# shinshoji01/Style-Restricted_GAN

Hardware: AMD Instinct MI355X
Metric: images/sec G+D+E train step, CelebA 128x128 bs=32/GPU (higher is better)
Workload: dtype f32; 1 GPU; SRGAN-nopretrain (03-train) G+D+E train step, 128x128, bs=32/GPU, k=5, fp32, E trainable (BASELINE configs[1]); global_batch=32, unrolled_k=5, parallelism=dp1, graph_fallback=False, graph_segments=1, ranks_seen=1, execution=hipGraph replay of the captured step

## Files before the change

include/srgan_hip.h:

```cpp
#ifndef SRGAN_HIP_H
#define SRGAN_HIP_H

#include <stddef.h>
#include <stdint.h>

#ifdef __cplusplus
extern "C" {
#endif

#define SRGAN_ABI_VERSION 1

enum { SRGAN_ACT_NONE = 0, SRGAN_ACT_RELU = 1, SRGAN_ACT_LRELU = 2 };
enum { SRGAN_PAD_ZERO = 0, SRGAN_PAD_REFLECT = 1 };
enum { SRGAN_CRIT_MSE = 0, SRGAN_CRIT_BCE = 1 };

int srgan_abi_version(void);
const char* srgan_last_error(void);

typedef struct srgan_conv_desc {
  int N, Hi, Wi, I;
  int Ho, Wo, O;
  int kh, kw, stride, pad;
  int pad_mode;
  long long sO, sI, sH, sW;
// ... 152 lines not shown
                       void* dst, int dst_bf16, int act, float slope, void* ws, size_t ws_bytes, void* stream);
int srgan_igemm16_wgrad(const srgan_conv_desc* d, const void* x, const void* dy, float* dw, void* ws, size_t ws_bytes, void* stream);
int srgan_conv2d_io_applicable(const srgan_conv_desc* d, int act);
int srgan_conv2d_io_fwd(const srgan_conv_desc* d, const void* x, int x_bf16, const void* packed, const float* bias, void* y, int y_bf16,
                        int act, float slope, void* ws, size_t ws_bytes, void* stream);
int srgan_conv2d_io_dgrad(const srgan_conv_desc* d, const void* dy, int dy_bf16, const void* packed, void* dx, int dx_bf16, void* ws,
                          size_t ws_bytes, void* stream);
int srgan_act_bwd_io(const void* y, int y_bf16, const void* dy, int dy_bf16, void* dx, int dx_bf16, long long n, int act, float slope,
                     void* stream);
int srgan_instnorm_slab_applicable(int N, int HW, int C);
int srgan_instnorm_slab_fwd_io(const void* x, int x_bf16, const float* scale, const float* shift, const float* res, void* y,
                               int y_bf16, float* mean, float* rstd, int N, int HW, int C, float eps, int act, float slope,
                               void* stream);
int srgan_instnorm_slab_bwd_io(const void* x, int x_bf16, const void* dy, int dy_bf16, const float* scale, const float* shift,
                               const float* mean, const float* rstd, void* dx, int dx_bf16, float* dscale, float* dshift, int N,
                               int HW, int C, int act, float slope, void* stream);
int srgan_instnorm_io_applicable(int N, int HW, int C);
int srgan_instnorm_fwd_io(const void* x, int x_bf16, const float* scale, const float* shift, const float* res, void* y, int y_bf16,
                          float* mean, float* rstd, int N, int HW, int C, float eps, int act, float slope, void* ws, size_t ws_bytes,
                          void* stream);
int srgan_instnorm_bwd_io(const void* x, int x_bf16, const void* dy, int dy_bf16, const float* scale, const float* shift,
                          const float* mean, const float* rstd, void* dx, int dx_bf16, float* dscale, float* dshift, int N, int HW,
                          int C, int act, float slope, void* ws, size_t ws_bytes, void* stream);

int srgan_nchw_to_nhwc(const float* x, float* y, int N, int C, int H, int W, void* stream);
int srgan_nhwc_to_nchw(const float* x, float* y, int N, int C, int H, int W, void* stream);

int srgan_mse_const(const float* o, long long n, float target, float weight, float* loss, float* d_o, void* stream);
int srgan_crit_const(const float* o, long long n, float target, float weight, int kind, float* loss, float* d_o, void* stream);
int srgan_softmax_mse(const float* z, const long long* label, int B, int n_class, float weight,
                      float* q, float* loss, float* dz, void* stream);
int srgan_softmax_crit(const float* z, const long long* label, int B, int n_class, float weight, int kind,
                       float* q, float* loss, float* dz, void* stream);
int srgan_softmax_xent(const float* z, const long long* label, int B, int n_class, float weight, float* loss,
                       float* dz, void* stream);
size_t srgan_l1_workspace(long long n);
int srgan_l1_mean(const float* a, const float* b, long long n, float weight, float* loss,
                  float* da, float* db, void* ws, size_t ws_bytes, void* stream);
int srgan_latent_losses(const float* mu, int B, int d, float n_batch, const float* hist_target, int bins,
                        float range_max, float sigma, float w_bkl, float w_corr, float w_hist,
                        float* vals, float* dmu, float* corr_out , void* stream);
int srgan_d_losses(const float* const* o, const long long* per_row, const float* const* z, int n_scales, int rows,
                   int rows_first, int n_class, const long long* label, float t_first, float t_rest, float w_class,
                   float* vals, float* const* d_o, float* const* dz, void* stream);
int srgan_d_losses_crit(const float* const* o, const long long* per_row, const float* const* z, int n_scales, int rows,
                        int rows_first, int n_class, const long long* label, float t_first, float t_rest, float w_class,
// ... 87 lines not shown
```

style-restricted_gan_amd/csrc/norm.hip:

```cpp
#include <algorithm>
#include <cstdlib>
#include <cstring>
#include "common.h"

namespace srgan {

constexpr int NORM_CH = 32;
constexpr int NORM_ROWS = 8;

template <bool B16>
__device__ __forceinline__ f32x4 ld4(const void* base, size_t idx) {
  if constexpr (B16) return __builtin_convertvector(*reinterpret_cast<const bf16x4*>(static_cast<const __bf16*>(base) + idx), f32x4);
  else return *reinterpret_cast<const f32x4*>(static_cast<const float*>(base) + idx);
}
template <bool B16>
__device__ __forceinline__ void st4(void* base, size_t idx, f32x4 v) {
  if constexpr (B16) *reinterpret_cast<bf16x4*>(static_cast<__bf16*>(base) + idx) = __builtin_convertvector(v, bf16x4);
  else *reinterpret_cast<f32x4*>(static_cast<float*>(base) + idx) = v;
}


template <bool B16>
__device__ __forceinline__ void ld8(const void* base, size_t idx, f32x4& lo, f32x4& hi) {
  if constexpr (B16) {
// ... 277 lines not shown
  for (int s = 0; s < S; ++s) {
    const float2 p = part[((size_t)n * S + s) * C + c];
    a += p.x;
    b += p.y;
  }
  stats_finish(a, b, x[(size_t)n * HW * C + c], HW, eps, &mean[idx], &rstd[idx]);
}

__device__ __forceinline__ void sum_partials4(const float2* __restrict__ part, int n, int S, int C, int c, f32x4* a, f32x4* b) {
  f32x4 sa = {0.f, 0.f, 0.f, 0.f}, sb = {0.f, 0.f, 0.f, 0.f};
  for (int s = 0; s < S; ++s) {
    const f32x4* q = reinterpret_cast<const f32x4*>(part + ((size_t)n * S + s) * C + c);
    const f32x4 lo = q[0], hi = q[1];
    sa[0] += lo[0]; sb[0] += lo[1]; sa[1] += lo[2]; sb[1] += lo[3];
    sa[2] += hi[0]; sb[2] += hi[1]; sa[3] += hi[2]; sb[3] += hi[3];
  }
  *a = sa;
  *b = sb;
}

template <bool V4>
__global__ void in_apply(const float* __restrict__ x, const float* __restrict__ scale, const float* __restrict__ shift,
                         const float* __restrict__ res, const float* __restrict__ mean, const float* __restrict__ rstd,
                         float* __restrict__ y, long long total, int HWC, int C, int act, float slope) {
  constexpr int W = V4 ? 4 : 1;
  for (long long i = ((long long)blockIdx.x * blockDim.x + threadIdx.x) * W; i < total;
       i += (long long)gridDim.x * blockDim.x * W) {
    const int n = (int)(i / HWC);
    const int c = (int)(i % C);
    float xv[W], rv[W], o[W];
    if constexpr (V4) {
      *reinterpret_cast<f32x4*>(xv) = *reinterpret_cast<const f32x4*>(x + i);
      if (res) *reinterpret_cast<f32x4*>(rv) = *reinterpret_cast<const f32x4*>(res + i);
    } else {
      xv[0] = x[i];
      if (res) rv[0] = res[i];
    }
#pragma unroll
    for (int k = 0; k < W; ++k) {
      const int nc = n * C + c + k;
      float v = (xv[k] - mean[nc]) * rstd[nc];
      if (scale) v = v * scale[nc] + shift[nc];
      v = apply_act(v, act, slope);
      if (res) v += rv[k];
      o[k] = v;
    }
    if constexpr (V4) *reinterpret_cast<f32x4*>(y + i) = *reinterpret_cast<const f32x4*>(o);
    else y[i] = o[0];
  }
}

template <bool X16 = false, bool Y16 = false>
__global__ __launch_bounds__(256) void in_apply_pow2(const void* __restrict__ x, const float* __restrict__ scale,
                                                     const float* __restrict__ shift, const float* __restrict__ res,
                                                     float* __restrict__ mean, float* __restrict__ rstd,
                                                     void* __restrict__ y, int HWC4, int C, int act, float slope,
                                                     const float2* __restrict__ part, int S, int HW, float eps) {
  const int n = blockIdx.y;
  const int c = (threadIdx.x * 4) % C;
  const int nc = n * C + c;
  f32x4 mu, rs;
  if (part) {
    f32x4 a, b;
    sum_partials4(part, n, S, C, c, &a, &b);
    const f32x4 x0 = ld4<X16>(x, (size_t)n * HWC4 * 4 + c);
#pragma unroll
    for (int e = 0; e < 4; ++e) {
      float m1, r1;
      stats_finish(a[e], b[e], x0[e], HW, eps, &m1, &r1);
      mu[e] = m1;
      rs[e] = r1;
    }
    if (blockIdx.x == 0 && threadIdx.x * 4 < C) {
      *reinterpret_cast<f32x4*>(mean + nc) = mu;
      *reinterpret_cast<f32x4*>(rstd + nc) = rs;
    }
  } else {
    mu = *reinterpret_cast<const f32x4*>(mean + nc);
    rs = *reinterpret_cast<const f32x4*>(rstd + nc);
  }
  f32x4 sc = {1.f, 1.f, 1.f, 1.f}, sf = {0.f, 0.f, 0.f, 0.f};
  if (scale) {
    sc = *reinterpret_cast<const f32x4*>(scale + nc);
    sf = *reinterpret_cast<const f32x4*>(shift + nc);
  }
  const size_t base = (size_t)n * HWC4;
  const f32x4* rp = res ? reinterpret_cast<const f32x4*>(res) + base : nullptr;
  auto xat = [&](int j) __attribute__((always_inline)) { return ld4<X16>(x, (base + j) * 4); };
  auto yput = [&](int j, f32x4 v) __attribute__((always_inline)) { st4<Y16>(y, (base + j) * 4, v); };
  auto one = [&](f32x4 xv, f32x4 rv) __attribute__((always_inline)) {
    f32x4 v = ((xv - mu) * rs) * sc + sf;
#pragma unroll
    for (int k = 0; k < 4; ++k) v[k] = apply_act(v[k], act, slope);
    return rp ? v + rv : v;
  };
  const int step = gridDim.x * 256;
  int j = blockIdx.x * 256 + threadIdx.x;
  const f32x4 zero = {0.f, 0.f, 0.f, 0.f};
  for (; j + 3 * step < HWC4; j += 4 * step) {
    const f32x4 x0v = xat(j), x1v = xat(j + step), x2v = xat(j + 2 * step), x3v = xat(j + 3 * step);
    f32x4 r0 = zero, r1 = zero, r2 = zero, r3 = zero;
    if (rp) { r0 = rp[j]; r1 = rp[j + step]; r2 = rp[j + 2 * step]; r3 = rp[j + 3 * step]; }
    yput(j, one(x0v, r0));
    yput(j + step, one(x1v, r1));
    yput(j + 2 * step, one(x2v, r2));
    yput(j + 3 * step, one(x3v, r3));
  }
  for (; j < HWC4; j += step) yput(j, one(xat(j), rp ? rp[j] : zero));
}

template <bool X16 = false, bool G16 = false, bool D16 = false>
// ... 562 lines not shown
    else if (rows <= 2) SRGAN_FWD_SLAB(2);
    else if (rows <= 4) SRGAN_FWD_SLAB(4);
    else if (rows <= 8) SRGAN_FWD_SLAB(8);
    else SRGAN_FWD_SLAB(16);
#undef SRGAN_FWD_SLAB
    prof_end(tok, st);
    return check_launch("instnorm_fwd (slab)");
  }
  float2* part = reinterpret_cast<float2*>(ws);
  dim3 g((C + NORM_CH - 1) / NORM_CH, S, N);
  {
    ProfToken tok = prof_begin(30, tbytes, st);
    if ((C & 3) == 0) hipLaunchKernelGGL(in_stats_partial_v4<false>, g, dim3(256), 0, st, (const void*)x, part, HW, C, S, rps);
    else hipLaunchKernelGGL(in_stats_partial, g, dim3(256), 0, st, x, part, HW, C, S, rps);
    prof_end(tok, st);
  }
  const long long total = (long long)N * HW * C;
  const bool fuse_final = (const float*)y != x && (const float*)y != res;
  if (pow2_fast(C, HW) && fuse_final) {
    const int hwc4 = HW * C / 4;
    dim3 g2((unsigned)apply_grid(hwc4, N), (unsigned)N);
    ProfToken tok = prof_begin(31, (res ? 3.0 : 2.0) * tbytes, st);
    hipLaunchKernelGGL((in_apply_pow2<false, false>), g2, dim3(256), 0, st, (const void*)x, scale, shift, res, mean, rstd, (void*)y, hwc4, C, act, slope,
                       (const float2*)part, S, HW, eps);
    prof_end(tok, st);
    return check_launch("instnorm_fwd");
  }
  hipLaunchKernelGGL(in_stats_final, dim3((N * C + 255) / 256), dim3(256), 0, st, x, (const float2*)part, mean, rstd, N, HW, C, S, eps);
  if (pow2_fast(C, HW)) {
    const int hwc4 = HW * C / 4;
    dim3 g2((unsigned)apply_grid(hwc4, N), (unsigned)N);
    hipLaunchKernelGGL((in_apply_pow2<false, false>), g2, dim3(256), 0, st, (const void*)x, scale, shift, res, mean, rstd, (void*)y, hwc4, C, act, slope,
                       (const float2*)nullptr, 0, HW, eps);
  } else if ((C & 3) == 0) {
    unsigned blocks = (unsigned)std::min<long long>(ceil_div(total / 4, 256), 8192);
    hipLaunchKernelGGL(in_apply<true>, dim3(blocks), dim3(256), 0, st, x, scale, shift, res, mean, rstd, y, total, HW * C, C, act, slope);
  } else {
    unsigned blocks = (unsigned)std::min<long long>(ceil_div(total, 256), 8192);
    hipLaunchKernelGGL(in_apply<false>, dim3(blocks), dim3(256), 0, st, x, scale, shift, res, mean, rstd, y, total, HW * C, C, act, slope);
  }
  return check_launch("instnorm_fwd");
}

extern "C" int srgan_instnorm_bwd(const float* x, const float* dy, const float* scale, const float* shift,
                                  const float* mean, const float* rstd, float* dx, float* dscale, float* dshift,
                                  int N, int HW, int C, int act, float slope, void* ws, size_t ws_bytes, void* stream) {
  SRGAN_REQUIRE(x && dy && mean && rstd && dx && dscale && dshift, "instnorm_bwd: null pointer");
  SRGAN_REQUIRE((scale == nullptr) == (shift == nullptr), "instnorm_bwd: scale and shift go together");
  hipStream_t st = as_stream(stream);
  int S, rps;
  plan_split(N, HW, C, S, rps);
  SRGAN_REQUIRE(ws && ws_bytes >= (size_t)N * S * C * sizeof(float2), "instnorm_bwd: workspace too small");
  const double tbytes = (double)N * HW * C * sizeof(float);
  if (slab_fast(N, HW, C)) {
    const dim3 gs((unsigned)(C / 16), (unsigned)N);
    const int rows = (HW + 63) / 64;
#define SRGAN_BWD_SLAB(R) hipLaunchKernelGGL(in_bwd_slab<R>, gs, dim3(256), 0, st, x, dy, scale, shift, mean, rstd, dx, dscale, dshift, HW, C, act, slope, slab_remap())
    ProfToken tok = prof_begin(35, 3.0 * tbytes, st);
    if (rows <= 1) SRGAN_BWD_SLAB(1);
    else if (rows <= 2) SRGAN_BWD_SLAB(2);
    else if (rows <= 4) SRGAN_BWD_SLAB(4);
    else if (rows <= 8) SRGAN_BWD_SLAB(8);
// ... 115 lines not shown
  SRGAN_REQUIRE(x && y && mean && rstd, "instnorm_fwd_io: null pointer");
  SRGAN_REQUIRE(srgan_instnorm_io_applicable(N, HW, C), "instnorm_fwd_io: shape not served (srgan_instnorm_io_applicable)");
  SRGAN_REQUIRE(x != y && (const void*)res != (const void*)y, "instnorm_fwd_io: in-place calls are not supported");
  SRGAN_REQUIRE(!(res && y_bf16), "instnorm_fwd_io: the skip tensor is added to an fp32 result only");
  if (slab_fast(N, HW, C)) return srgan_instnorm_slab_fwd_io(x, x_bf16, scale, shift, res, y, y_bf16, mean, rstd, N, HW, C, eps, act, slope, stream);
  SRGAN_REQUIRE((scale == nullptr) == (shift == nullptr), "instnorm_fwd_io: scale and shift go together");
  hipStream_t st = as_stream(stream);
  int S, rps;
  plan_split(N, HW, C, S, rps);
  SRGAN_REQUIRE(ws && ws_bytes >= (size_t)N * S * C * sizeof(float2), "instnorm_fwd_io: workspace too small (srgan_instnorm_workspace)");
  const double ebytes = (double)N * HW * C;
  float2* part = reinterpret_cast<float2*>(ws);
  dim3 g((C + NORM_CH - 1) / NORM_CH, S, N);
  {
    ProfToken tok = prof_begin(30, ebytes * (x_bf16 ? 2 : 4), st);
    if (x_bf16 && (C & 63) == 0) hipLaunchKernelGGL(in_stats_partial_v8, dim3(C / 64, S, N), dim3(256), 0, st, x, part, HW, C, S, rps);
    else if (x_bf16) hipLaunchKernelGGL(in_stats_partial_v4<true>, g, dim3(256), 0, st, x, part, HW, C, S, rps);
    else hipLaunchKernelGGL(in_stats_partial_v4<false>, g, dim3(256), 0, st, x, part, HW, C, S, rps);
    prof_end(tok, st);
  }
  const int hwc4 = HW * C / 4;
  dim3 g2((unsigned)apply_grid(hwc4, N), (unsigned)N);
  ProfToken tok = prof_begin(31, ebytes * ((x_bf16 ? 2 : 4) + (y_bf16 ? 2 : 4) + (res ? 4 : 0)), st);
#define SRGAN_APPLY_IO(A, B) hipLaunchKernelGGL((in_apply_pow2<A, B>), g2, dim3(256), 0, st, x, scale, shift, res, mean, rstd, y, hwc4, C, act, slope, (const float2*)part, S, HW, eps)
  if (x_bf16 && y_bf16) SRGAN_APPLY_IO(true, true);
  else if (x_bf16) SRGAN_APPLY_IO(true, false);
  else if (y_bf16) SRGAN_APPLY_IO(false, true);
  else SRGAN_APPLY_IO(false, false);
#undef SRGAN_APPLY_IO
  prof_end(tok, st);
  return check_launch("instnorm_fwd_io");
}

extern "C" int srgan_instnorm_bwd_io(const void* x, int x_bf16, const void* dy, int dy_bf16, const float* scale, const float* shift,
                                     const float* mean, const float* rstd, void* dx, int dx_bf16, float* dscale, float* dshift, int N,
                                     int HW, int C, int act, float slope, void* ws, size_t ws_bytes, void* stream) {
  SRGAN_REQUIRE(x && dy && mean && rstd && dx && dscale && dshift, "instnorm_bwd_io: null pointer");
  SRGAN_REQUIRE(srgan_instnorm_io_applicable(N, HW, C), "instnorm_bwd_io: shape not served (srgan_instnorm_io_applicable)");
  SRGAN_REQUIRE((x_bf16 != 0) == (dx_bf16 != 0), "instnorm_bwd_io: the input gradient has the input's type");
  if (slab_fast(N, HW, C)) {
    return srgan_instnorm_slab_bwd_io(x, x_bf16, dy, dy_bf16, scale, shift, mean, rstd, dx, dx_bf16, dscale, dshift, N, HW, C, act, slope, stream);
  }
  SRGAN_REQUIRE((scale == nullptr) == (shift == nullptr), "instnorm_bwd_io: scale and shift go together");
  hipStream_t st = as_stream(stream);
  int S, rps;
  plan_split(N, HW, C, S, rps);
  SRGAN_REQUIRE(ws && ws_bytes >= (size_t)N * S * C * sizeof(float2), "instnorm_bwd_io: workspace too small (srgan_instnorm_workspace)");
  const double ebytes = (double)N * HW * C;
  const int xb = x_bf16 ? 2 : 4, gb = dy_bf16 ? 2 : 4;
  float2* part = reinterpret_cast<float2*>(ws);
  dim3 g((C + NORM_CH - 1) / NORM_CH, S, N);
  {
    ProfToken tok = prof_begin(32, ebytes * (xb + gb), st);
#define SRGAN_BPART_IO(A, B) hipLaunchKernelGGL((in_bwd_partial_v4<A, B>), g, dim3(256), 0, st, x, dy, scale, shift, mean, rstd, part, HW, C, S, rps, act, slope)
// ... 89 lines not shown
```

style-restricted_gan_amd/srgan_amd/_lib.py:

```python
import ctypes
import os
from ctypes import c_float, c_int, c_longlong, c_size_t, c_void_p, POINTER

_HERE = os.path.dirname(os.path.abspath(__file__))
LIB_PATH = os.environ.get("SRGAN_HIP_LIB") or os.path.join(_HERE, "libsrgan_hip.so")
EXPERIMENTS = bool(os.environ.get("SRGAN_HIP_LIB"))


def ab(name):
    return EXPERIMENTS and bool(os.environ.get(name))


def active_switches():
    out = {}
    if EXPERIMENTS:
        out["SRGAN_HIP_LIB"] = os.environ["SRGAN_HIP_LIB"]
        out.update({k: v for k, v in os.environ.items() if k.startswith("SRGAN_") and k != "SRGAN_HIP_LIB"})
    return out


class ConvDesc(ctypes.Structure):
    _fields_ = [("N", c_int), ("Hi", c_int), ("Wi", c_int), ("I", c_int),
                ("Ho", c_int), ("Wo", c_int), ("O", c_int),
                ("kh", c_int), ("kw", c_int), ("stride", c_int), ("pad", c_int),
# ... 18 lines not shown
    "srgan_conv2d_fwd": (c_int, [_DESC, P, P, P, P, c_int, c_float, P, c_size_t, P]),
    "srgan_conv2d_dgrad": (c_int, [_DESC, P, P, P, P, c_size_t, P]),
    "srgan_conv2d_packed_bytes": (c_size_t, [_DESC, c_int, c_int]),
    "srgan_conv2d_pack": (c_int, [_DESC, c_int, c_int, P, P, c_size_t, P]),
    "srgan_conv2d_packed_scratch": (c_size_t, [_DESC, c_int]),
    "srgan_conv2d_pack_signature": (ctypes.c_ulonglong, [_DESC, c_int, c_int]),
    "srgan_conv2d_fwd_packed": (c_int, [_DESC, P, P, P, P, c_int, c_float, P, c_size_t, P]),
    "srgan_conv2d_dgrad_packed": (c_int, [_DESC, P, P, P, P, c_size_t, P]),
    "srgan_conv2d_dgrad_packed_mask": (c_int, [_DESC, P, P, P, c_float, P, P, c_size_t, P]),
    "srgan_conv2d_dgrad_packed_add": (c_int, [_DESC, P, P, P, P, P, c_size_t, P]),
    "srgan_instnorm_conv_v_applicable": (c_int, [_DESC]),
    "srgan_instnorm_fwd_v": (c_int, [_DESC, P, P, P, P, P, P, c_size_t, c_float, c_int, c_float, P]),
    "srgan_conv2d_fwd_from_v": (c_int, [_DESC, P, P, P, P, c_int, c_float, P]),
    "srgan_instnorm_bwd_vz_applicable": (c_int, [_DESC]),
    "srgan_instnorm_bwd_vz_z_bytes": (c_size_t, [_DESC]),
    "srgan_instnorm_bwd_vz": (c_int, [_DESC, P, P, P, P, P, P, P, P, P, c_size_t, P, c_size_t, c_int, c_float, P]),
    "srgan_conv2d_dgrad_from_v": (c_int, [_DESC, P, P, P, P, P]),
    "srgan_conv2d_wgrad_vz": (c_int, [_DESC, P, P, P, P, c_size_t, P]),
    "srgan_halo16_applicable": (c_int, [_DESC]),
    "srgan_halo16s2_applicable": (c_int, [_DESC]),
    "srgan_instnorm_io_applicable": (c_int, [c_int, c_int, c_int]),
    "srgan_instnorm_fwd_io": (c_int, [P, c_int, P, P, P, P, c_int, P, P, c_int, c_int, c_int, c_float, c_int, c_float, P, c_size_t, P]),
    "srgan_instnorm_bwd_io": (c_int, [P, c_int, P, c_int, P, P, P, P, P, c_int, P, P, c_int, c_int, c_int, c_int, c_float, P, c_size_t, P]),
    "srgan_halo16_conv": (c_int, [_DESC, c_int, P, c_int, P, P, P, c_int, P]),
    "srgan_halo16_wgrad": (c_int, [_DESC, P, c_int, P, c_int, P, P, c_size_t, P]),
    "srgan_conv2d_io_applicable": (c_int, [_DESC, c_int]),
    "srgan_conv2d_io_fwd": (c_int, [_DESC, P, c_int, P, P, P, c_int, c_int, c_float, P, c_size_t, P]),
    "srgan_conv2d_io_dgrad": (c_int, [_DESC, P, c_int, P, P, c_int, P, c_size_t, P]),
    "srgan_act_bwd_io": (c_int, [P, c_int, P, c_int, P, c_int, c_longlong, c_int, c_float, P]),
    "srgan_igemm16_io_applicable": (c_int, [_DESC, c_int]),
    "srgan_igemm16_conv": (c_int, [_DESC, c_int, P, c_int, P, P, P, c_int, c_int, c_float, P, c_size_t, P]),
    "srgan_igemm16_wgrad": (c_int, [_DESC, P, P, P, P, c_size_t, P]),
    "srgan_instnorm_slab_applicable": (c_int, [c_int, c_int, c_int]),
    "srgan_instnorm_slab_fwd_io": (c_int, [P, c_int, P, P, P, P, c_int, P, P, c_int, c_int, c_int, c_float, c_int, c_float, P]),
    "srgan_instnorm_slab_bwd_io": (c_int, [P, c_int, P, c_int, P, P, P, P, P, c_int, P, P, c_int, c_int, c_int, c_int, c_float, P]),
    "srgan_set_wgrad_accumulate": (c_int, [c_int]),
    "srgan_wgrad_defer_begin": (c_int, [P, c_size_t, P]),
    "srgan_wgrad_defer_end": (c_int, []),
    "srgan_wgrad_defer_stats": (c_int, [POINTER(c_longlong), POINTER(c_longlong)]),
    "srgan_wgrad_defer_need": (c_int, [POINTER(c_longlong)]),
    "srgan_conv2d_wgrad": (c_int, [_DESC, P, P, P, P, P, c_size_t, P]),
    "srgan_conv2d_wgrad_v_bytes": (c_size_t, [_DESC]),
    "srgan_conv2d_wgrad_v": (c_int, [_DESC, P, P, P, P, P, c_size_t, P]),
    "srgan_instnorm_workspace": (c_size_t, [c_int, c_int, c_int]),
    "srgan_instnorm_fwd": (c_int, [P, P, P, P, P, P, P, c_int, c_int, c_int, c_float, c_int, c_float, P, c_size_t, P]),
    "srgan_instnorm_bwd": (c_int, [P, P, P, P, P, P, P, P, P, c_int, c_int, c_int, c_int, c_float, P, c_size_t, P]),
# ... 133 lines not shown
```

style-restricted_gan_amd/srgan_amd/model.py:

```python
import functools

import numpy as np
import os
import torch
import torch.nn as nn

from . import _lib, ops
from .ops import ACT_LRELU, ACT_NONE, ACT_RELU, PAD_REFLECT, PAD_ZERO

__all__ = ["CBINorm2d", "CBBNorm2d", "BatchNorm2d", "get_norm_layer", "per_sample", "SingleResidualBlock", "SingleGenerator",
           "SingleDiscriminator_original", "SingleDiscriminator_original_multi", "SingleDiscriminator_solo",
           "SingleDiscriminator_solo_multi", "BasicBlock", "Encoder_original", "BasicBlock_classification",
           "Encoder", "Encoder_classifier", "MinMax"]

D_SLOPE = 0.01
E_SLOPE = 0.2


class _Conv2d(nn.Conv2d):

    def forward(self, x, act=ACT_NONE, slope=0.0, in_slope=None, act_bwd_by_consumer=False, io16=None):
        if io16 is not None:
            return ops.conv2d_s2_io(x, self.weight, io16)
        mode = PAD_REFLECT if self.padding_mode == "reflect" else PAD_ZERO
# ... 354 lines not shown
        self.num_cls = num_cls
        k, s, p = 2 * reduce, reduce, int(reduce / 2)

        convs = [_Conv2d(nch_in, nch, kernel_size=7, stride=1, padding=3, bias=False)]
        cnorms = [c_norm_layer(nch)]
        for i in range(num_cls):
            convs.append(_Conv2d(nch * 2 ** i, nch * 2 ** (i + 1), kernel_size=k, stride=s, padding=p, bias=False))
            cnorms.append(c_norm_layer(nch * 2 ** (i + 1)))
        self.down_convs = nn.ModuleList(convs)
        self.down_cnorms = nn.ModuleList(cnorms)

        self.resBlocks = nn.Sequential(*[SingleResidualBlock(nch * 2 ** num_cls, c_norm_layer) for _ in range(res_num)])

        ups = [_ConvTranspose2d(nch * 2 ** num_cls, nch * 2 ** (num_cls - 1), kernel_size=k, stride=s, padding=p, bias=False)]
        norms = [norm_layer(nch * 2 ** (num_cls - 1))]
        for i in range(1, num_cls)[::-1]:
            ups.append(_ConvTranspose2d(nch * 2 ** i, nch * 2 ** (i - 1), kernel_size=k, stride=s, padding=p, bias=False))
            norms.append(norm_layer(nch * 2 ** (i - 1)))
        ups.append(_Conv2d(nch, nch_out, kernel_size=7, stride=1, padding=3, bias=False))
        self.up_convs = nn.ModuleList(ups)
        self.up_norms = nn.ModuleList(norms)
        self._per_sample = per_sample(self)

    def forward(self, x, c):
        if c.is_cuda and not _lib.ab("SRGAN_NO_CBIN_MULTI"):
            c = PrecomputedCon(c, list(self.down_cnorms) + [n for blk in self.resBlocks for n in (blk.cn1, blk.cn2)])
        n, _, h, w = x.shape
        io = [False] * (self.num_cls + 2)
        s16 = self._per_sample
        if s16 and x.is_cuda and ops.get_compute_dtype() == "bf16":
            hh, ww = h, w
            for i in range(1, self.num_cls + 1):
                cv = self.down_convs[i]
                probe = torch.empty((n, cv.in_channels, hh, ww), device="meta")
                io[i] = (cv.s2_io_applicable(probe) and ops.norm_io_applicable(n, cv.in_channels, hh, ww)
                         and ops.norm_io_applicable(n, cv.out_channels, hh // 2, ww // 2))
                hh, ww = hh // 2, ww // 2
        cv0, cvl = self.down_convs[0], self.up_convs[-1]
        rgb16 = [s16 and x.is_cuda and cv.kernel_size == (7, 7) and cv.bias is None and
                 ops.conv_act_io_applicable(n, cv.in_channels, h, w, cv.weight, ACT_NONE, 7, 1, 3) and
                 ops.norm_io_applicable(n, ch, h, w) for cv, ch in ((cv0, cv0.out_channels), (cvl, cvl.in_channels))]
        for i in range(self.num_cls + 1):
            if i == 0 and rgb16[0]:
                y = ops.conv2d_act_io(x, cv0.weight, ACT_NONE, 0.0, True, 7, 1, 3)
            else:
                y = self.down_convs[i](x, io16=True) if io[i] else self.down_convs[i](x)
            x = self.down_cnorms[i](y, c, ACT_RELU, out_bf16=io[i + 1])
        x = self.resBlocks([x, c])[0]
        n, _, h, w = x.shape
        iot = [False] * (self.num_cls + 1)
        nio = [False] * (self.num_cls + 1)
        if s16 and x.is_cuda and ops.get_compute_dtype() == "bf16":
            hh, ww = h, w
            for i in range(self.num_cls):
                cv = self.up_convs[i]
                probe = torch.empty((n, cv.in_channels, hh, ww), device="meta")
                nio[i] = ops.norm_io_applicable(n, cv.out_channels, 2 * hh, 2 * ww)
                iot[i] = cv.s2_io_applicable(probe) and nio[i]
                hh, ww = 2 * hh, 2 * ww
        for i in range(self.num_cls):
            y = self.up_convs[i](x, io16=True) if iot[i] else self.up_convs[i](x)
            x = self.up_norms[i](y, ACT_RELU, out_bf16=(iot[i + 1] and nio[i]) or (i == self.num_cls - 1 and rgb16[1] and nio[i]))
        if x.dtype == torch.bfloat16:
            return ops.tanh(ops.conv2d_act_io(x, cvl.weight, ACT_NONE, 0.0, False, 7, 1, 3))
        return ops.tanh(self.up_convs[-1](x))

# ... 339 lines not shown
```

style-restricted_gan_amd/srgan_amd/ops.py:

```python
import ctypes
import struct
import weakref

import torch
from torch.autograd import Function

from . import _lib
from ._lib import ConvDesc

ACT_NONE, ACT_RELU, ACT_LRELU = 0, 1, 2
PAD_ZERO, PAD_REFLECT = 0, 1

_workspaces = {}
import os as _os
_DEBUG_FRESH_WS = _lib.ab('SRGAN_DEBUG_FRESH_WS')
_DEBUG_CLONE = _lib.ab('SRGAN_DEBUG_CLONE')


def _require_gpu(t, what):
    if not t.is_cuda:
        raise _lib.SrganHipError(f"{what}: tensor is on {t.device}; srgan_amd runs on the MI355X HIP path only "
                                 "(no CPU fallback)")
    if t.dtype != torch.float32:
        raise _lib.SrganHipError(f"{what}: expected float32, got {t.dtype}")
# ... 1340 lines not shown
        dscale = torch.empty(n, c, dtype=torch.float32, device=x.device)
        dshift = torch.empty_like(dscale)
        nb = lib.srgan_instnorm_workspace(n, h * w, c)
        ws = workspace(x.device, nb)
        _lib.check(lib.srgan_instnorm_bwd_io(_ptr(x), _is16(x), _ptr(gy), _is16(gy), _ptr(scale), _ptr(shift), _ptr(mean), _ptr(rstd),
                                             _ptr(dx), _is16(dx), _ptr(dscale), _ptr(dshift), n, h * w, c, ctx.act, float(ctx.slope),
                                             _ptr(ws), nb, _stream()), "instnorm_bwd_io")
        has_aff = scale is not None
        return dx, dscale if has_aff else None, dshift if has_aff else None, None, None, None, None


def conv2d_s2_io(x, weight, out_bf16):
    return _ConvS2IoFn.apply(x, weight, bool(out_bf16))


def conv_transpose2d_io(x, weight, out_bf16):
    return _ConvT2IoFn.apply(x, weight, bool(out_bf16))


def instance_norm_act_io(x, scale, shift, act=ACT_NONE, slope=0.0, eps=1e-5, out_bf16=False):
    return _InstNormIoFn.apply(x, scale, shift, act, slope, eps, bool(out_bf16))




_NO_CONV_IO16 = _lib.ab("SRGAN_NO_CONV_IO16")


def conv_io_applicable(n, ci, hi, wi, weight, pad, pad_mode):
    if not (STORAGE_BF16 and _pack_cache_on and get_compute_dtype() == "bf16" and weight.is_cuda) or _NO_CONV_IO16:
        return False
    co, _, kh, kw = weight.shape
    ho, wo = hi + 2 * pad - kh + 1, wi + 2 * pad - kw + 1
    if ho < 1 or wo < 1:
        return False
    desc = _conv_desc(n, hi, wi, ci, ho, wo, co, kh, kw, 1, pad, pad_mode, weight)
    return bool(_lib.load().srgan_igemm16_io_applicable(ctypes.byref(desc), ACT_NONE))


def _to16(t):
    return t if t.dtype == torch.bfloat16 else t.to(torch.bfloat16)


class _ConvIoFn(Function):

    @staticmethod
# ... 921 lines not shown
```

style-restricted_gan_amd/srgan_amd/trainer.py:

```python
import contextlib
import gc
import os

import numpy as np
import torch
import torch.nn as nn
import torch.optim as optim

from . import _lib, dp, ema, ops, spectral
from .losses import class_encode, criterion_kind, get_domainloss_D, get_loss_D, has_fused_kind, histogram_imitation
from .model import SingleGenerator, _cpu_normal_like, _is_batch_stat, _is_synced, batch_stats_synced, host_to_device, per_sample
from .optim import Adam

__all__ = ["SRGAN_training", "SingleGAN_training"]


@contextlib.contextmanager
def _frozen(params):
    flags = [(p, p.requires_grad) for p in params]
    for p, _ in flags:
        p.requires_grad_(False)
    try:
        yield
    finally:
        for p, f in flags:
            p.requires_grad_(f)


class SRGAN_training():

    def __init__(self, net, opt, criterion, lbd, unrolled_k, device, ref_label,
                 batch_size=64, encoded_feature="latent", ndim=8):
        self.G, self.D, self.E = net[0].to(device), net[1].to(device), net[2].to(device)
        self.optG, self.optD, self.optE = opt[0], opt[1], opt[2]
        self.scheG, self.scheD, self.scheE = None, None, None
        self.criterion, self.criterion_class = criterion
        self.lbd = lbd
        self.k = unrolled_k
        self.device = device
        self.ref_label = ref_label
        self.n_batch = batch_size
        self.encoded_feature = encoded_feature
        self.ndim = ndim
        self.source_image = None
        self.target_image = None
        self.recon_image = None
        self.label = None
        self.c_rand = None
        self.enc_info = None
        self.target_cenc = None
        if lbd["hist"] > 0:
            self.hi = histogram_imitation(device)
        self.loss_terms = {}
        self._reducers = {}
        self.noise_fn = torch.randn
        self._graph = None
        self._g_active = False
        self._ema = None
        self.G_ema = self.E_ema = None
        self._ema_scope = False
        ref = np.asarray(ref_label)
        self._ref_is_onehot = ref.ndim == 2 and ref.shape[0] == ref.shape[1] and np.array_equal(ref, np.eye(ref.shape[0]))
        self._g_per_sample = per_sample(dp.unwrap(self.G))
        self._e_per_sample = per_sample(dp.unwrap(self.E))
        if dp.world_size() > 1 and not (batch_stats_synced(dp.unwrap(self.G)) and batch_stats_synced(dp.unwrap(self.E))):
            raise NotImplementedError(
                "SRGAN_training: G / E hold batch-statistics norms (norm_type='batch') and a process group has "
                f"{dp.world_size()} ranks; nn.DataParallel gives per-replica statistics and rank-0 running buffers, which this "
                "package does not build (one process, or norm_type='instance'). Statistics of the global batch are an opt-in: "
                "mark both networks with dp.sync_batch_stats(net).")
        self._sn()

    def opt_sche_initialization(self, lr=[0.0001, 0.0001, 0.0001]):
        lr_G, lr_D, lr_E = lr
        if self.optG is None:
            self.optG = Adam(self.G.parameters(), lr=lr_G, betas=(0.5, 0.999))
        self.scheG = optim.lr_scheduler.ExponentialLR(self.optG, gamma=0.95)
        if self.optD is None:
            self.optD = Adam(self.D.parameters(), lr=lr_D, betas=(0.5, 0.999))
        self.scheD = optim.lr_scheduler.ExponentialLR(self.optD, gamma=0.95)
        if self.optE is None:
            self.optE = Adam(self.E.parameters(), lr=lr_E, betas=(0.5, 0.999))
        self.scheE = optim.lr_scheduler.ExponentialLR(self.optE, gamma=0.95)
# ... 343 lines not shown
                    errG_ex = errG_ex + errG_idt_reg * (L["idt_reg"] * (L["idt"] / L["cycle"]))
                    terms["errG_idt_reg"] = errG_idt_reg
            self._reduce_arm("G", self.optG)
            with ops.fused_param_grads(not dp.hooks_need_live_grads(), self.device):
                errG_ex.backward()
        redG = self._reduce_start("G", self.optG)
        if redG is not None:
            redG.finish()
        self._step(self.optG)

        self.recon_image = recon_image.detach()
        self.loss_terms.update({k: v.detach() for k, v in terms.items()})
        with torch.no_grad():
            errG = ops.lincomb([(errG, 1.0), (errG_ex, 1.0)])
        return [errG, errE_output.detach()]

    def UnrolledUpdate(self):
        errorD = None
        src, k = self.source_image, self.k
        nb = src.shape[0]
        noises = [self._noise("randn", nb) for _ in range(k)]
        oh = self._onehot("target")
        if dp.is_distributed():
            def translate(i):
                if i < k - 1:
                    with torch.no_grad():
                        return self.G(src, torch.cat([oh, noises[i]], 1)), noises[i]
                return self.G(src, torch.cat([oh, noises[i]], 1)), noises[i]

            fake = translate(0)
            for i in range(k):
                nxt = (lambda j=i + 1: translate(j)) if i + 1 < k else None
                out = self.update_D(_fake=fake, _next_fake=nxt, _defer=(i == k - 1))
                errD, fake = out if nxt is not None else (out, None)
                if i == 0:
                    errorD = errD.detach()
            errorG, errorE = self.update_GandE()
            self._ema_update()
            return [errorG, errorD, errorE]
        fakes = []
        if k > 1 and isinstance(dp.unwrap(self.G), SingleGenerator) and self._g_per_sample:
            Gm = dp.unwrap(self.G)
            widest = max(int(Gm.down_convs[0].weight.shape[0]), 3) * src.shape[2] * src.shape[3] * 4
            per_group = max(1, min(k - 1, (((1 << 32) - (1 << 26)) // widest) // nb))
            with torch.no_grad():
                for lo in range(0, k - 1, per_group):
                    zs = noises[lo:min(lo + per_group, k - 1)]
                    c_all = torch.cat([torch.cat([oh, z], 1) for z in zs], 0)
                    imgs = self.G(ops.cat_batch([src] * len(zs)) if len(zs) > 1 else src, c_all)
                    fakes += [(imgs[i * nb:(i + 1) * nb], z) for i, z in enumerate(zs)]
        elif k > 1:
            with torch.no_grad():
                fakes = [(self.G(src, torch.cat([oh, z], 1)), z) for z in noises[:-1]]
        fakes.append((self.G(src, torch.cat([oh, noises[-1]], 1)), noises[-1]))
        for i in range(k):
            errD = self.update_D(_fake=fakes[i])
            fakes[i] = None
            if i == 0:
                errorD = errD.detach()
        errorG, errorE = self.update_GandE()
        self._ema_update()
        return [errorG, errorD, errorE]

    def _ema_update(self):
        if self._ema is not None:
            self._ema.update()

    def train(self, source_image, label):
        if self._ema_scope:
            raise RuntimeError("SRGAN_training.train() inside ema_weights(): self.G / self.E are the averaged copies there")
        self.label = label
        self.loss_terms = {}
        g = self._graph
        sn = self._sn()
        if sn is not None:
            sn._ensure()
        if g is not None and g.accepts(source_image, label):
# ... 188 lines not shown
        return (tuple(source_image.shape), dev(label["source"]), dev(label["target"]))

    def _fingerprint(self):
        sg = self.sg
        fp = [sg.k, sg.n_batch, sg.ndim, sg.encoded_feature, tuple(sorted((k, float(v)) for k, v in sg.lbd.items())),
              type(sg.criterion), type(sg.criterion_class), np.asarray(sg.ref_label, dtype=np.float64).tobytes()]
        fp.append((has_fused_kind(sg.criterion, "gan"), has_fused_kind(sg.criterion_class, "class")))
        for opt in (sg.optG, sg.optD, sg.optE):
            fp.append(id(opt))
            for g in getattr(opt, "param_groups", ()):
                fp.append((tuple(g["betas"]), float(g["eps"])))
                for p in g["params"]:
                    st = opt.state.get(p) or {}
                    m, v = st.get("exp_avg"), st.get("exp_avg_sq")
                    fp.append((id(p), m.data_ptr() if m is not None else 0, v.data_ptr() if v is not None else 0))
        fp.append(tuple((id(p), p.data_ptr(), p.requires_grad) for p in self._all_params()))
        fp.append(tuple((id(m), m.training, m.momentum, m.eps, m.track_running_stats, _is_synced(m)) for net in (sg.G, sg.E)
                        for m in net.modules() if _is_batch_stat(m)))
        cur = getattr(sg, "_ema", None)
        fp.append(cur.fingerprint() if cur is not None else None)
        fp.append(tuple(opt.grad_guard_fingerprint() if isinstance(opt, Adam) else None for opt in (sg.optG, sg.optD, sg.optE)))
        sn = sg._sn() if hasattr(sg, "_sn") else None
        fp.append(sn.fingerprint() if sn is not None else None)
        return tuple(fp)

    def _opt_steps(self):
        sg = self.sg
        return [[int(opt.state[p]["step"]) if len(opt.state.get(p) or {}) else -1 for g in opt.param_groups for p in g["params"]]
                for opt in (sg.optG, sg.optD, sg.optE)]

    def _drop(self):
        self.graph, self.key, self._keep, self._baked, self._steps = None, None, None, None, None
        self.x = self.noise = self.out = None

    def _local_mode(self, source_image, label):
        if dp.is_distributed() and self.unsupported_reason() is self.SEGMENTED_SYNC:
            if self.graph is not None:
                self._drop()
            return 0
        if self.graph is not None:
            stale = self._epoch != ops.structure_epoch()
            if not stale and (self._baked != self._fingerprint() or self._steps != self._opt_steps()):
                stale = True
                reason = self.unsupported_reason()
                if reason:
                    raise NotImplementedError("SRGAN_training graph mode: " + reason)
# ... 472 lines not shown
```

Baseline: 529.5 images/sec.

## Share generator stem conv across k noise samples and broadcast instnorm

The first 7x7 conv of the generator depends only on the source image, not the noise/style code, so it is computed once per step and reused for all k translations. Under no_grad, a new broadcast instance-norm kernel computes statistics on the n_src stem outputs only and applies the per-sample CBIN scale/shift to the replicated batch, without materialising the concatenated input. This removes (k-1) redundant stem convolutions and the stem stats/copy traffic, at the cost of extra code paths and a new kernel variant with modular indexing.

```diff
diff --git a/include/srgan_hip.h b/include/srgan_hip.h
--- a/include/srgan_hip.h
+++ b/include/srgan_hip.h
@@ -198,6 +198,10 @@
 int srgan_instnorm_bwd_io(const void* x, int x_bf16, const void* dy, int dy_bf16, const float* scale, const float* shift,
                           const float* mean, const float* rstd, void* dx, int dx_bf16, float* dscale, float* dshift, int N, int HW,
                           int C, int act, float slope, void* ws, size_t ws_bytes, void* stream);
+int srgan_instnorm_bcast_applicable(int n_src, int N, int HW, int C, int x_bf16, int y_bf16);
+int srgan_instnorm_fwd_bcast(const void* x, int x_bf16, int n_src, const float* scale, const float* shift, void* y, int y_bf16,
+                             float* mean, float* rstd, int N, int HW, int C, float eps, int act, float slope, void* ws,
+                             size_t ws_bytes, void* stream);
 
 int srgan_nchw_to_nhwc(const float* x, float* y, int N, int C, int H, int W, void* stream);
 int srgan_nhwc_to_nchw(const float* x, float* y, int N, int C, int H, int W, void* stream);
diff --git a/style-restricted_gan_amd/csrc/norm.hip b/style-restricted_gan_amd/csrc/norm.hip
--- a/style-restricted_gan_amd/csrc/norm.hip
+++ b/style-restricted_gan_amd/csrc/norm.hip
@@ -323,24 +323,26 @@
 template <bool V4>
 __global__ void in_apply(const float* __restrict__ x, const float* __restrict__ scale, const float* __restrict__ shift,
                          const float* __restrict__ res, const float* __restrict__ mean, const float* __restrict__ rstd,
-                         float* __restrict__ y, long long total, int HWC, int C, int act, float slope) {
+                         float* __restrict__ y, long long total, int HWC, int C, int act, float slope, int n_src) {
   constexpr int W = V4 ? 4 : 1;
   for (long long i = ((long long)blockIdx.x * blockDim.x + threadIdx.x) * W; i < total;
        i += (long long)gridDim.x * blockDim.x * W) {
     const int n = (int)(i / HWC);
     const int c = (int)(i % C);
+    const int ns = n_src ? n % n_src : n;
+    const long long xi = i - (long long)(n - ns) * HWC;
     float xv[W], rv[W], o[W];
     if constexpr (V4) {
-      *reinterpret_cast<f32x4*>(xv) = *reinterpret_cast<const f32x4*>(x + i);
+      *reinterpret_cast<f32x4*>(xv) = *reinterpret_cast<const f32x4*>(x + xi);
       if (res) *reinterpret_cast<f32x4*>(rv) = *reinterpret_cast<const f32x4*>(res + i);
     } else {
-      xv[0] = x[i];
+      xv[0] = x[xi];
       if (res) rv[0] = res[i];
     }
 #pragma unroll
     for (int k = 0; k < W; ++k) {
-      const int nc = n * C + c + k;
-      float v = (xv[k] - mean[nc]) * rstd[nc];
+      const int nc = n * C + c + k, ncs = ns * C + c + k;
+      float v = (xv[k] - mean[ncs]) * rstd[ncs];
       if (scale) v = v * scale[nc] + shift[nc];
       v = apply_act(v, act, slope);
       if (res) v += rv[k];
@@ -356,15 +358,16 @@
                                                      const float* __restrict__ shift, const float* __restrict__ res,
                                                      float* __restrict__ mean, float* __restrict__ rstd,
                                                      void* __restrict__ y, int HWC4, int C, int act, float slope,
-                                                     const float2* __restrict__ part, int S, int HW, float eps) {
+                                                     const float2* __restrict__ part, int S, int HW, float eps, int n_src) {
   const int n = blockIdx.y;
+  const int ns = n_src ? n % n_src : n;
   const int c = (threadIdx.x * 4) % C;
   const int nc = n * C + c;
   f32x4 mu, rs;
   if (part) {
     f32x4 a, b;
-    sum_partials4(part, n, S, C, c, &a, &b);
-    const f32x4 x0 = ld4<X16>(x, (size_t)n * HWC4 * 4 + c);
+    sum_partials4(part, ns, S, C, c, &a, &b);
+    const f32x4 x0 = ld4<X16>(x, (size_t)ns * HWC4 * 4 + c);
 #pragma unroll
     for (int e = 0; e < 4; ++e) {
       float m1, r1;
@@ -377,17 +380,17 @@
       *reinterpret_cast<f32x4*>(rstd + nc) = rs;
     }
   } else {
-    mu = *reinterpret_cast<const f32x4*>(mean + nc);
-    rs = *reinterpret_cast<const f32x4*>(rstd + nc);
+    mu = *reinterpret_cast<const f32x4*>(mean + ns * C + c);
+    rs = *reinterpret_cast<const f32x4*>(rstd + ns * C + c);
   }
   f32x4 sc = {1.f, 1.f, 1.f, 1.f}, sf = {0.f, 0.f, 0.f, 0.f};
   if (scale) {
     sc = *reinterpret_cast<const f32x4*>(scale + nc);
     sf = *reinterpret_cast<const f32x4*>(shift + nc);
   }
-  const size_t base = (size_t)n * HWC4;
+  const size_t base = (size_t)n * HWC4, xbase = (size_t)ns * HWC4;
   const f32x4* rp = res ? reinterpret_cast<const f32x4*>(res) + base : nullptr;
-  auto xat = [&](int j) __attribute__((always_inline)) { return ld4<X16>(x, (base + j) * 4); };
+  auto xat = [&](int j) __attribute__((always_inline)) { return ld4<X16>(x, (xbase + j) * 4); };
   auto yput = [&](int j, f32x4 v) __attribute__((always_inline)) { st4<Y16>(y, (base + j) * 4, v); };
   auto one = [&](f32x4 xv, f32x4 rv) __attribute__((always_inline)) {
     f32x4 v = ((xv - mu) * rs) * sc + sf;
@@ -996,7 +999,7 @@
     dim3 g2((unsigned)apply_grid(hwc4, N), (unsigned)N);
     ProfToken tok = prof_begin(31, (res ? 3.0 : 2.0) * tbytes, st);
     hipLaunchKernelGGL((in_apply_pow2<false, false>), g2, dim3(256), 0, st, (const void*)x, scale, shift, res, mean, rstd, (void*)y, hwc4, C, act, slope,
-                       (const float2*)part, S, HW, eps);
+                       (const float2*)part, S, HW, eps, 0);
     prof_end(tok, st);
     return check_launch("instnorm_fwd");
   }
@@ -1005,13 +1008,13 @@
     const int hwc4 = HW * C / 4;
     dim3 g2((unsigned)apply_grid(hwc4, N), (unsigned)N);
     hipLaunchKernelGGL((in_apply_pow2<false, false>), g2, dim3(256), 0, st, (const void*)x, scale, shift, res, mean, rstd, (void*)y, hwc4, C, act, slope,
-                       (const float2*)nullptr, 0, HW, eps);
+                       (const float2*)nullptr, 0, HW, eps, 0);
   } else if ((C & 3) == 0) {
     unsigned blocks = (unsigned)std::min<long long>(ceil_div(total / 4, 256), 8192);
-    hipLaunchKernelGGL(in_apply<true>, dim3(blocks), dim3(256), 0, st, x, scale, shift, res, mean, rstd, y, total, HW * C, C, act, slope);
+    hipLaunchKernelGGL(in_apply<true>, dim3(blocks), dim3(256), 0, st, x, scale, shift, res, mean, rstd, y, total, HW * C, C, act, slope, 0);
   } else {
     unsigned blocks = (unsigned)std::min<long long>(ceil_div(total, 256), 8192);
-    hipLaunchKernelGGL(in_apply<false>, dim3(blocks), dim3(256), 0, st, x, scale, shift, res, mean, rstd, y, total, HW * C, C, act, slope);
+    hipLaunchKernelGGL(in_apply<false>, dim3(blocks), dim3(256), 0, st, x, scale, shift, res, mean, rstd, y, total, HW * C, C, act, slope, 0);
   }
   return check_launch("instnorm_fwd");
 }
@@ -1173,7 +1176,7 @@
   const int hwc4 = HW * C / 4;
   dim3 g2((unsigned)apply_grid(hwc4, N), (unsigned)N);
   ProfToken tok = prof_begin(31, ebytes * ((x_bf16 ? 2 : 4) + (y_bf16 ? 2 : 4) + (res ? 4 : 0)), st);
-#define SRGAN_APPLY_IO(A, B) hipLaunchKernelGGL((in_apply_pow2<A, B>), g2, dim3(256), 0, st, x, scale, shift, res, mean, rstd, y, hwc4, C, act, slope, (const float2*)part, S, HW, eps)
+#define SRGAN_APPLY_IO(A, B) hipLaunchKernelGGL((in_apply_pow2<A, B>), g2, dim3(256), 0, st, x, scale, shift, res, mean, rstd, y, hwc4, C, act, slope, (const float2*)part, S, HW, eps, 0)
   if (x_bf16 && y_bf16) SRGAN_APPLY_IO(true, true);
   else if (x_bf16) SRGAN_APPLY_IO(true, false);
   else if (y_bf16) SRGAN_APPLY_IO(false, true);
@@ -1181,6 +1184,63 @@
 #undef SRGAN_APPLY_IO
   prof_end(tok, st);
   return check_launch("instnorm_fwd_io");
+}
+
+extern "C" int srgan_instnorm_bcast_applicable(int n_src, int N, int HW, int C, int x_bf16, int y_bf16) {
+  if (n_src <= 0 || N <= 0 || HW <= 0 || C <= 0 || N % n_src != 0 || slab_fast(N, HW, C)) return 0;
+  if (x_bf16 || y_bf16) return ((C & 3) == 0 && pow2_fast(C, HW)) ? 1 : 0;
+  return 1;
+}
+
+extern "C" int srgan_instnorm_fwd_bcast(const void* x, int x_bf16, int n_src, const float* scale, const float* shift, void* y,
+                                        int y_bf16, float* mean, float* rstd, int N, int HW, int C, float eps, int act, float slope,
+                                        void* ws, size_t ws_bytes, void* stream) {
+  SRGAN_REQUIRE(x && y && mean && rstd, "instnorm_fwd_bcast: null pointer");
+  SRGAN_REQUIRE(x != y, "instnorm_fwd_bcast: in-place calls are not supported");
+  SRGAN_REQUIRE((scale == nullptr) == (shift == nullptr), "instnorm_fwd_bcast: scale and shift go together");
+  SRGAN_REQUIRE(srgan_instnorm_bcast_applicable(n_src, N, HW, C, x_bf16, y_bf16),
+                "instnorm_fwd_bcast: shape not served (srgan_instnorm_bcast_applicable)");
+  hipStream_t st = as_stream(stream);
+  int S, rps;
+  plan_split(N, HW, C, S, rps);
+  SRGAN_REQUIRE(ws && ws_bytes >= (size_t)n_src * S * C * sizeof(float2), "instnorm_fwd_bcast: workspace too small (srgan_instnorm_workspace)");
+  const double ebytes = (double)HW * C;
+  const int xb = x_bf16 ? 2 : 4, yb = y_bf16 ? 2 : 4;
+  float2* part = reinterpret_cast<float2*>(ws);
+  dim3 g((C + NORM_CH - 1) / NORM_CH, S, n_src);
+  {
+    ProfToken tok = prof_begin(30, ebytes * n_src * xb, st);
+    if (x_bf16 && (C & 63) == 0) hipLaunchKernelGGL(in_stats_partial_v8, dim3(C / 64, S, n_src), dim3(256), 0, st, x, part, HW, C, S, rps);
+    else if (x_bf16) hipLaunchKernelGGL(in_stats_partial_v4<true>, g, dim3(256), 0, st, x, part, HW, C, S, rps);
+    else if ((C & 3) == 0) hipLaunchKernelGGL(in_stats_partial_v4<false>, g, dim3(256), 0, st, x, part, HW, C, S, rps);
+    else hipLaunchKernelGGL(in_stats_partial, g, dim3(256), 0, st, (const float*)x, part, HW, C, S, rps);
+    prof_end(tok, st);
+  }
+  if (pow2_fast(C, HW)) {
+    const int hwc4 = HW * C / 4;
+    dim3 g2((unsigned)apply_grid(hwc4, N), (unsigned)N);
+    ProfToken tok = prof_begin(31, ebytes * (n_src * xb + N * yb), st);
+#define SRGAN_APPLY_BC(A, B) hipLaunchKernelGGL((in_apply_pow2<A, B>), g2, dim3(256), 0, st, x, scale, shift, (const float*)nullptr, mean, rstd, y, hwc4, C, act, slope, (const float2*)part, S, HW, eps, n_src)
+    if (x_bf16 && y_bf16) SRGAN_APPLY_BC(true, true);
+    else if (x_bf16) SRGAN_APPLY_BC(true, false);
+    else if (y_bf16) SRGAN_APPLY_BC(false, true);
+    else SRGAN_APPLY_BC(false, false);
+#undef SRGAN_APPLY_BC
+    prof_end(tok, st);
+    return check_launch("instnorm_fwd_bcast");
+  }
+  const float* xf = static_cast<const float*>(x);
+  float* yf = static_cast<float*>(y);
+  const long long total = (long long)N * HW * C;
+  hipLaunchKernelGGL(in_stats_final, dim3((n_src * C + 255) / 256), dim3(256), 0, st, xf, (const float2*)part, mean, rstd, n_src, HW, C, S, eps);
+  if ((C & 3) == 0) {
+    unsigned blocks = (unsigned)std::min<long long>(ceil_div(total / 4, 256), 8192);
+    hipLaunchKernelGGL(in_apply<true>, dim3(blocks), dim3(256), 0, st, xf, scale, shift, (const float*)nullptr, mean, rstd, yf, total, HW * C, C, act, slope, n_src);
+  } else {
+    unsigned blocks = (unsigned)std::min<long long>(ceil_div(total, 256), 8192);
+    hipLaunchKernelGGL(in_apply<false>, dim3(blocks), dim3(256), 0, st, xf, scale, shift, (const float*)nullptr, mean, rstd, yf, total, HW * C, C, act, slope, n_src);
+  }
+  return check_launch("instnorm_fwd_bcast");
 }
 
 extern "C" int srgan_instnorm_bwd_io(const void* x, int x_bf16, const void* dy, int dy_bf16, const float* scale, const float* shift,
diff --git a/style-restricted_gan_amd/srgan_amd/_lib.py b/style-restricted_gan_amd/srgan_amd/_lib.py
--- a/style-restricted_gan_amd/srgan_amd/_lib.py
+++ b/style-restricted_gan_amd/srgan_amd/_lib.py
@@ -64,6 +64,8 @@
     "srgan_instnorm_io_applicable": (c_int, [c_int, c_int, c_int]),
     "srgan_instnorm_fwd_io": (c_int, [P, c_int, P, P, P, P, c_int, P, P, c_int, c_int, c_int, c_float, c_int, c_float, P, c_size_t, P]),
     "srgan_instnorm_bwd_io": (c_int, [P, c_int, P, c_int, P, P, P, P, P, c_int, P, P, c_int, c_int, c_int, c_int, c_float, P, c_size_t, P]),
+    "srgan_instnorm_bcast_applicable": (c_int, [c_int] * 6),
+    "srgan_instnorm_fwd_bcast": (c_int, [P, c_int, c_int, P, P, P, c_int, P, P, c_int, c_int, c_int, c_float, c_int, c_float, P, c_size_t, P]),
     "srgan_halo16_conv": (c_int, [_DESC, c_int, P, c_int, P, P, P, c_int, P]),
     "srgan_halo16_wgrad": (c_int, [_DESC, P, c_int, P, c_int, P, P, c_size_t, P]),
     "srgan_conv2d_io_applicable": (c_int, [_DESC, c_int]),
diff --git a/style-restricted_gan_amd/srgan_amd/model.py b/style-restricted_gan_amd/srgan_amd/model.py
--- a/style-restricted_gan_amd/srgan_amd/model.py
+++ b/style-restricted_gan_amd/srgan_amd/model.py
@@ -400,10 +400,40 @@
         self.up_norms = nn.ModuleList(norms)
         self._per_sample = per_sample(self)
 
-    def forward(self, x, c):
+    def _rgb16(self, cv, ch, n, h, w, like):
+        return bool(self._per_sample and like.is_cuda and cv.kernel_size == (7, 7) and cv.bias is None and
+                    ops.conv_act_io_applicable(n, cv.in_channels, h, w, cv.weight, ACT_NONE, 7, 1, 3) and
+                    ops.norm_io_applicable(n, ch, h, w))
+
+    def stem(self, x):
+        n, _, h, w = x.shape
+        cv0 = self.down_convs[0]
+        if self._rgb16(cv0, cv0.out_channels, n, h, w, x):
+            return ops.conv2d_act_io(x, cv0.weight, ACT_NONE, 0.0, True, 7, 1, 3)
+        return cv0(x)
+
+    def stem_shareable(self, x, n_out):
+        n, _, h, w = x.shape
+        cv0, cn0 = self.down_convs[0], self.down_cnorms[0]
+        if not (self._per_sample and x.is_cuda and isinstance(cn0, CBINorm2d) and n_out % n == 0):
+            return False
+        s16 = self._rgb16(cv0, cv0.out_channels, n, h, w, x)
+        if s16 != self._rgb16(cv0, cv0.out_channels, n_out, h, w, x):
+            return False
+        outs = (False, True) if ops.get_compute_dtype() == "bf16" else (False,)
+        return all(ops.instance_norm_bcast_applicable(n, cv0.out_channels, h, w, n_out, s16, o16) for o16 in outs)
+
+    def forward(self, x, c, stem=None):
+        rep = 1
+        if stem is not None:
+            rep = c.shape[0] // stem.shape[0]
+            if rep * stem.shape[0] != c.shape[0]:
+                raise ValueError("SingleGenerator: the batch of the style codes is no multiple of the stem's")
+            x = stem
         if c.is_cuda and not _lib.ab("SRGAN_NO_CBIN_MULTI"):
             c = PrecomputedCon(c, list(self.down_cnorms) + [n for blk in self.resBlocks for n in (blk.cn1, blk.cn2)])
         n, _, h, w = x.shape
+        n *= rep
         io = [False] * (self.num_cls + 2)
         s16 = self._per_sample
         if s16 and x.is_cuda and ops.get_compute_dtype() == "bf16":
@@ -415,11 +445,17 @@
                          and ops.norm_io_applicable(n, cv.out_channels, hh // 2, ww // 2))
                 hh, ww = hh // 2, ww // 2
         cv0, cvl = self.down_convs[0], self.up_convs[-1]
-        rgb16 = [s16 and x.is_cuda and cv.kernel_size == (7, 7) and cv.bias is None and
-                 ops.conv_act_io_applicable(n, cv.in_channels, h, w, cv.weight, ACT_NONE, 7, 1, 3) and
-                 ops.norm_io_applicable(n, ch, h, w) for cv, ch in ((cv0, cv0.out_channels), (cvl, cvl.in_channels))]
+        rgb16 = [self._rgb16(cv, ch, n, h, w, x) for cv, ch in ((cv0, cv0.out_channels), (cvl, cvl.in_channels))]
         for i in range(self.num_cls + 1):
-            if i == 0 and rgb16[0]:
+            if i == 0 and stem is not None:
+                cn0 = self.down_cnorms[0]
+                if rep > 1 and not torch.is_grad_enabled() and isinstance(cn0, CBINorm2d) \
+                        and ops.instance_norm_bcast_applicable(n // rep, stem.shape[1], h, w, n, stem.dtype == torch.bfloat16, io[1]):
+                    scale, shift = cn0.scale_shift(c, stem.device)
+                    x = ops.instance_norm_act_bcast(stem, scale, shift, ACT_RELU, 0.0, cn0.eps, io[1])
+                    continue
+                y = ops.cat_batch([stem] * rep) if rep > 1 else stem
+            elif i == 0 and rgb16[0]:
                 y = ops.conv2d_act_io(x, cv0.weight, ACT_NONE, 0.0, True, 7, 1, 3)
             else:
                 y = self.down_convs[i](x, io16=True) if io[i] else self.down_convs[i](x)
diff --git a/style-restricted_gan_amd/srgan_amd/ops.py b/style-restricted_gan_amd/srgan_amd/ops.py
--- a/style-restricted_gan_amd/srgan_amd/ops.py
+++ b/style-restricted_gan_amd/srgan_amd/ops.py
@@ -1386,6 +1386,27 @@
     return _InstNormIoFn.apply(x, scale, shift, act, slope, eps, bool(out_bf16))
 
 
+def instance_norm_bcast_applicable(n, c, h, w, n_out, x_bf16=False, out_bf16=False):
+    return bool(_lib.load().srgan_instnorm_bcast_applicable(n, n_out, h * w, c, int(bool(x_bf16)), int(bool(out_bf16))))
+
+
+def instance_norm_act_bcast(x, scale, shift, act=ACT_NONE, slope=0.0, eps=1e-5, out_bf16=False):
+    _require_gpu(scale, "instance_norm_act_bcast")
+    x = to_nhwc(x.detach())
+    n, c, h, w = x.shape
+    n_out = scale.shape[0]
+    lib = _lib.load()
+    y = nhwc_empty(n_out, c, h, w, x.device, torch.bfloat16 if out_bf16 else torch.float32)
+    mean = torch.empty(n_out * c, dtype=torch.float32, device=x.device)
+    rstd = torch.empty_like(mean)
+    nb = lib.srgan_instnorm_workspace(n_out, h * w, c)
+    ws = workspace(x.device, nb)
+    _lib.check(lib.srgan_instnorm_fwd_bcast(_ptr(x), _is16(x), n, _ptr(scale.detach()), _ptr(shift.detach()), _ptr(y), _is16(y),
+                                            _ptr(mean), _ptr(rstd), n_out, h * w, c, float(eps), act, float(slope), _ptr(ws), nb,
+                                            _stream()), "instnorm_fwd_bcast")
+    return y
+
+
 
 
 _NO_CONV_IO16 = _lib.ab("SRGAN_NO_CONV_IO16")
diff --git a/style-restricted_gan_amd/srgan_amd/trainer.py b/style-restricted_gan_amd/srgan_amd/trainer.py
--- a/style-restricted_gan_amd/srgan_amd/trainer.py
+++ b/style-restricted_gan_amd/srgan_amd/trainer.py
@@ -13,6 +13,12 @@
 from .optim import Adam
 
 __all__ = ["SRGAN_training", "SingleGAN_training"]
+
+
+def _stem_arg(stem, detach=False):
+    if stem is None:
+        return {}
+    return {"stem": stem.detach() if detach else stem}
 
 
 @contextlib.contextmanager
@@ -59,6 +65,7 @@
         self._ema = None
         self.G_ema = self.E_ema = None
         self._ema_scope = False
+        self.share_stem = True
         ref = np.asarray(ref_label)
         self._ref_is_onehot = ref.ndim == 2 and ref.shape[0] == ref.shape[1] and np.array_equal(ref, np.eye(ref.shape[0]))
         self._g_per_sample = per_sample(dp.unwrap(self.G))
@@ -448,11 +455,14 @@
         noises = [self._noise("randn", nb) for _ in range(k)]
         oh = self._onehot("target")
         if dp.is_distributed():
+            Gm = dp.unwrap(self.G)
+            stem = Gm.stem(src) if self.share_stem and k > 1 and isinstance(Gm, SingleGenerator) and src.is_cuda else None
+
             def translate(i):
                 if i < k - 1:
                     with torch.no_grad():
-                        return self.G(src, torch.cat([oh, noises[i]], 1)), noises[i]
-                return self.G(src, torch.cat([oh, noises[i]], 1)), noises[i]
+                        return self.G(src, torch.cat([oh, noises[i]], 1), **_stem_arg(stem, detach=True)), noises[i]
+                return self.G(src, torch.cat([oh, noises[i]], 1), **_stem_arg(stem)), noises[i]
 
             fake = translate(0)
             for i in range(k):
@@ -464,21 +474,26 @@
             errorG, errorE = self.update_GandE()
             self._ema_update()
             return [errorG, errorD, errorE]
-        fakes = []
+        fakes, stem = [], None
         if k > 1 and isinstance(dp.unwrap(self.G), SingleGenerator) and self._g_per_sample:
             Gm = dp.unwrap(self.G)
             widest = max(int(Gm.down_convs[0].weight.shape[0]), 3) * src.shape[2] * src.shape[3] * 4
             per_group = max(1, min(k - 1, (((1 << 32) - (1 << 26)) // widest) // nb))
+            groups = [noises[lo:min(lo + per_group, k - 1)] for lo in range(0, k - 1, per_group)]
+            if self.share_stem and all(Gm.stem_shareable(src, len(zs) * nb) for zs in groups):
+                stem = Gm.stem(src)
             with torch.no_grad():
-                for lo in range(0, k - 1, per_group):
-                    zs = noises[lo:min(lo + per_group, k - 1)]
+                for zs in groups:
                     c_all = torch.cat([torch.cat([oh, z], 1) for z in zs], 0)
-                    imgs = self.G(ops.cat_batch([src] * len(zs)) if len(zs) > 1 else src, c_all)
+                    if stem is not None:
+                        imgs = self.G(src, c_all, stem=stem.detach())
+                    else:
+                        imgs = self.G(ops.cat_batch([src] * len(zs)) if len(zs) > 1 else src, c_all)
                     fakes += [(imgs[i * nb:(i + 1) * nb], z) for i, z in enumerate(zs)]
         elif k > 1:
             with torch.no_grad():
                 fakes = [(self.G(src, torch.cat([oh, z], 1)), z) for z in noises[:-1]]
-        fakes.append((self.G(src, torch.cat([oh, noises[-1]], 1)), noises[-1]))
+        fakes.append((self.G(src, torch.cat([oh, noises[-1]], 1), **_stem_arg(stem)), noises[-1]))
         for i in range(k):
             errD = self.update_D(_fake=fakes[i])
             fakes[i] = None
@@ -713,6 +728,7 @@
         fp.append(tuple(opt.grad_guard_fingerprint() if isinstance(opt, Adam) else None for opt in (sg.optG, sg.optD, sg.optE)))
         sn = sg._sn() if hasattr(sg, "_sn") else None
         fp.append(sn.fingerprint() if sn is not None else None)
+        fp.append(bool(getattr(sg, "share_stem", False)))
         return tuple(fp)
 
     def _opt_steps(self):
```

Result: no change. 534.3 images/sec, median of 6 (+0.9%).
